# sunkafei/coffeedb

Hardware: AMD Instinct MI355X
Metric: sa_build_GiB_per_s (higher is better)
Workload: dtype u64

## Files before the change

coffeedb_amd/csrc/capi.hip:

```cpp
#include <dirent.h>

#include <algorithm>
#include <chrono>
#include <condition_variable>
#include <cstdlib>
#include <cstring>
#include <thread>

#include "../../include/coffeedb_gpu.h"
#include "index_impl.h"

using namespace cdb;

namespace {

double wall_ms() {
    using namespace std::chrono;
    return duration<double, std::milli>(steady_clock::now().time_since_epoch()).count();
}

void set_error(Index& ix, const char* msg) {
    std::lock_guard<std::mutex> g(ix.err_mu);
    ix.err = msg;
}
// ... 1467 lines not shown
        out->nrows = r.nrows;
        out->nhits = r.nhits;
        out->d_row_ptr = ix.q_rowptr.as<uint64_t>();
        out->d_ids = ix.q_ids.as<int64_t>();
        out->d_counts = ix.q_counts.as<int64_t>();
        if (hits) {
            hits->d_hit_ptr = ix.q_hitptr.as<uint64_t>();
            hits->d_offsets = ix.q_hitoff.as<uint64_t>();
        }
        ix.qstats.query_ms = wall_ms() - t0;
        ix.qstats.nhits = r.nhits;
        ix.qstats.nrows = r.nrows;
    });
}
}

int cdb_query_batch_device(cdb_index* h, const void* d_blob, const uint64_t* d_offsets, uint64_t npat,
                           uint64_t blob_bytes, cdb_device_result* out) {
    (void)blob_bytes;
    return query_batch_device_impl(h, d_blob, d_offsets, npat, out, nullptr);
}

int cdb_query_batch_offsets_device(cdb_index* h, const void* d_blob, const uint64_t* d_offsets, uint64_t npat,
                                   uint64_t blob_bytes, cdb_device_result* out, cdb_device_hits* hits) {
    (void)blob_bytes;
    if (!hits) return CDB_E_INVALID;
    return query_batch_device_impl(h, d_blob, d_offsets, npat, out, hits);
}

uint64_t cdb_size(const cdb_index* h) { return h ? h->ix.size : 0; }
uint64_t cdb_bits(const cdb_index* h) { return h ? h->ix.bits : 0; }
uint64_t cdb_mask(const cdb_index* h) { return h ? h->ix.mask : 0; }
int cdb_sa_width(const cdb_index* h) { return h ? h->ix.width : 0; }

int cdb_sa_copy(cdb_index* h, void* host_out, uint64_t capacity_bytes) {
    if (!h || !host_out) return CDB_E_INVALID;
    return guarded(h, [&] {
        Index& ix = h->ix;
        std::lock_guard<std::mutex> g(ix.mu);
        DeviceScope dscope(ix);
        const uint64_t need = ix.size * (uint64_t)ix.width;
        if (capacity_bytes < need) throw Error("cdb_sa_copy: buffer too small");
        if (need && ix.sa_packed) {
            DevBuf chunk;
            const uint64_t per = std::min<uint64_t>(ix.size, 32ull << 20);
            chunk.alloc(per * 8);
            for (uint64_t first = 0; first < ix.size; first += per) {
                const uint64_t cnt = std::min<uint64_t>(per, ix.size - first);
                sa_expand(ix, first, cnt, chunk.as<uint64_t>());
                CDB_HIP(hipMemcpyAsync(static_cast<char*>(host_out) + first * 8, chunk.p, cnt * 8, hipMemcpyDeviceToHost, ix.stream));
                CDB_HIP(hipStreamSynchronize(ix.stream));
            }
        } else if (need) {
            CDB_HIP(hipMemcpyAsync(host_out, ix.d_sa.p, need, hipMemcpyDeviceToHost, ix.stream));
            CDB_HIP(hipStreamSynchronize(ix.stream));
        }
    });
}

int cdb_set_option(cdb_index* h, const char* name, int64_t value) {
    if (!h || !name) return CDB_E_INVALID;
    Index& ix = h->ix;
    for (const char* o : {"fast_search", "key_directory", "single_query", "search_lanes", "keep_keys", "reference_compat"})
        if (!std::strcmp(name, o)) {
            std::lock_guard<std::mutex> g(ix.mu);
            query_resident_stop(ix);
        }
    if (!std::strcmp(name, "profile")) ix.prof.enabled = value != 0;
    else if (!std::strcmp(name, "reference_compat")) ix.reference_compat = value != 0;
    else if (!std::strcmp(name, "force_doubling")) ix.force_doubling = value != 0;
    else if (!std::strcmp(name, "initial_passes")) ix.initial_passes = (int)value;
    else if (!std::strcmp(name, "sort_variant")) ix.sort_variant = (int)value;
    else if (!std::strcmp(name, "keyhist3")) ix.keyhist3 = value != 0;
    else if (!std::strcmp(name, "key_symbols")) ix.key_symbols = (int)value;
    else if (!std::strcmp(name, "msd_first")) ix.msd_first = value != 0;
    else if (!std::strcmp(name, "msd_pair")) ix.msd_pair = value != 0;
    else if (!std::strcmp(name, "overlap_paircount")) ix.overlap_paircount = value != 0;
    else if (!std::strcmp(name, "key_directory")) { ix.key_directory = value != 0; ix.h_keydir.clear(); ix.keydir_tried = false; }
    else if (!std::strcmp(name, "fuse_records")) ix.fuse_records = value != 0;
    else if (!std::strcmp(name, "sweep_records")) ix.sweep_records = value != 0;
    else if (!std::strcmp(name, "partial_symbol")) ix.partial_symbol = value != 0;
    else if (!std::strcmp(name, "group_sort")) ix.group_sort = value != 0;
    else if (!std::strcmp(name, "list_rounds")) ix.list_rounds = value != 0;
    else if (!std::strcmp(name, "fuse_pairclass")) ix.fuse_pairclass = value != 0;
    else if (!std::strcmp(name, "group_sort_cap")) ix.group_sort_cap = (int)std::max<int64_t>(1, std::min<int64_t>(value, 1 << 20));
    else if (!std::strcmp(name, "vl_keys")) ix.vl_keys = value < 0 ? 0 : (value > 56 ? 56 : (int)value);
    else if (!std::strcmp(name, "pack_sa")) ix.pack_sa = value != 0;
    else if (!std::strcmp(name, "key_cost_model")) ix.key_cost_model = value != 0;
    else if (!std::strcmp(name, "gen_prebased")) ix.gen_prebased = value != 0;
    else if (!std::strcmp(name, "pack_entries")) ix.pack_entries = value != 0;
    else if (!std::strcmp(name, "segmented_sort")) ix.segmented_sort = value != 0;
    else if (!std::strcmp(name, "fold_root")) ix.fold_root = value != 0;
    else if (!std::strcmp(name, "fold_depth1")) ix.fold_depth1 = value != 0;
    else if (!std::strcmp(name, "flags_in_last_pass")) ix.flags_in_last_pass = value != 0;
    else if (!std::strcmp(name, "search_lanes")) ix.search_lanes = (value == 1 || value == 8) ? (int)value : 0;
    else if (!std::strcmp(name, "digit_bits")) ix.digit_bits = (int)value;
    else if (!std::strcmp(name, "fuse_keygen")) ix.fuse_keygen = value != 0;
    else if (!std::strcmp(name, "force_big_path")) ix.force_big_path = value != 0;
    else if (!std::strcmp(name, "debug_fail_build")) ix.debug_fail_build = value != 0;
    else if (!std::strcmp(name, "debug_no_segcap")) ix.debug_no_segcap = value != 0;
    else if (!std::strcmp(name, "debug_starve_group")) ix.debug_starve_group = (int)value;
    else if (!std::strcmp(name, "self_check")) ix.self_check = value < 0 ? 0 : value > 3 ? 3 : (int)value;
    else if (!std::strcmp(name, "premap_generation")) ix.premap_generation = value != 0;
    else if (!std::strcmp(name, "proof_cancel")) {
        if (value) proof_stop(ix);
    }
    else if (!std::strcmp(name, "debug_damage_after_build")) ix.debug_damage_after_build = value < 0 ? 0 : (uint64_t)value;
    else if (!std::strcmp(name, "debug_fail_self_check")) ix.debug_fail_self_check = value != 0;
    else if (!std::strcmp(name, "plain_tile_order")) ix.rws.plain_order = value != 0;
    else if (!std::strcmp(name, "key_coding")) ix.key_coding = (int)value;
    else if (!std::strcmp(name, "narrow_keys")) ix.narrow_keys = value != 0;
    else if (!std::strcmp(name, "single_query")) ix.use_single_query = value != 0;
    else if (!std::strcmp(name, "resident_query")) {
        std::lock_guard<std::mutex> g(ix.mu);
        if (value != 1) query_resident_stop(ix);
        ix.resident_mode = value <= 0 ? 0 : value == 1 ? 1 : 2;
        ix.resident_query = ix.resident_mode == 1;
        ix.single_streak = 0;
    }
    else if (!std::strcmp(name, "bucket_group_limit")) ix.bucket_group_limit = (uint64_t)value;
    else if (!std::strcmp(name, "query_hit_budget"))
        ix.query_hit_budget = value > 0 ? std::min<uint64_t>((uint64_t)value, 1ull << 31) : 1;
    else if (!std::strcmp(name, "coalesce_queries")) ix.coalesce_queries = value != 0;
    else if (!std::strcmp(name, "fast_search")) ix.use_fast_search = value != 0;
    else if (!std::strcmp(name, "wave_rows")) ix.use_wave_rows = value != 0;
    else if (!std::strcmp(name, "keep_keys")) ix.keep_keys = value != 0;
    else {
        set_error(ix, (std::string("unknown option: ") + name).c_str());
        return CDB_E_INVALID;
    }
    return CDB_OK;
}

int cdb_get_stat(const cdb_index* h, const char* name, double* value) {
    if (!h || !name || !value) return CDB_E_INVALID;
    const BuildStats& b = h->ix.bstats;
    const QueryStats& q = h->ix.qstats;
    struct { const char* n; double v; } tab[] = {
        {"build_ms", b.build_ms}, {"alloc_ms", b.alloc_ms}, {"free_ms", b.free_ms}, {"rounds", (double)b.rounds}, {"ext_rounds", (double)b.ext_rounds},
        {"dbl_rounds", (double)b.dbl_rounds}, {"unresolved_after_initial", (double)b.unresolved_initial},
        {"unresolved_max", (double)b.unresolved_max}, {"sort_passes", (double)b.sort_passes},
        {"sort_passes_skipped", (double)b.sort_passes_skipped}, {"isa_built", (double)b.isa_built}, {"fused_keygen", (double)b.fused_keygen}, {"dense_keys", (double)b.dense_keys}, {"key_layout", (double)b.key_layout}, {"bucketed", (double)b.bucketed}, {"bucket_groups", (double)b.bucket_groups}, {"segmented", (double)b.segmented}, {"fused_records", (double)b.fused_records}, {"sweep_records", (double)b.sweep_records}, {"vl_key_bits", (double)b.vl_key_bits}, {"partial_levels", (double)b.partial_levels}, {"list_rounds", (double)b.list_rounds}, {"pairclass_fused", (double)b.pairclass_fused}, {"group_sorts", (double)b.group_sorts}, {"group_sort_fallbacks", (double)b.group_sort_fallbacks}, {"vl_avg_len", b.vl_avg_len}, {"vl_rate", b.vl_rate}, {"vl_est_unresolved", b.vl_est_unresolved}, {"fixed_est_unresolved", b.fixed_est_unresolved}, {"gen_prebased", (double)b.gen_prebased}, {"root_folded", (double)b.root_folded}, {"flags_in_last_pass", (double)b.flags_in_last_pass}, {"msd_first", (double)b.msd_first}, {"bucket_low_digits", (double)b.bucket_low_digits}, {"key_directory_cells", h->ix.h_keydir.empty() ? 0.0 : (double)(h->ix.h_keydir.size() - 1)}, {"group_fallbacks", (double)h->ix.group_fallbacks}, {"dense_key_retries", (double)h->ix.dense_key_retries}, {"self_check_fallbacks", (double)h->ix.self_check_fallbacks}, {"sa_packed", h->ix.sa_packed ? 1.0 : 0.0}, {"sa_bytes_per_entry", h->ix.sa_packed ? 5.0 : (double)h->ix.width}, {"self_check_pairs", (double)h->ix.self_check_pairs}, {"self_check_ms", h->ix.self_check_ms}, {"self_check_coverage", h->ix.size > 1 ? (double)h->ix.self_check_pairs / (double)(h->ix.size - 1) : 0.0},
        {"order_proved", (h->ix.proof.state.load() == 2 || h->ix.proof.state.load() == 3 || (h->ix.self_check == 2 && h->ix.width != 0)) ? 1.0 : 0.0},
        {"proof_state", (double)h->ix.proof.state.load()}, {"proof_ms", h->ix.proof.ms}, {"proof_repair_ms", h->ix.proof.repair_ms},
        {"proof_pairs", (double)h->ix.proof.pairs}, {"proof_bad_pairs", (double)h->ix.proof.found[0]}, {"proof_invalid_entries", (double)h->ix.proof.found[1]}, {"proof_skipped_pairs", (double)h->ix.proof.skipped}, {"proof_mixed_pairs", (double)h->ix.proof.mixed},
        {"proof_runs", (double)h->ix.proof.runs}, {"pool_big_mallocs", (double)DevPool::get().big_mallocs()}, {"premap_ms", h->ix.proof.premap_ms}, {"premap_bytes", (double)h->ix.proof.premap_bytes},
        {"key_symbols", (double)b.key_symbols}, {"symbol_bits", (double)b.symbol_bits},
        {"alphabet", (double)b.alphabet}, {"digit_bits", (double)b.digit_bits}, {"final_depth", (double)b.final_depth}, {"compat_rotations", (double)b.compat_rotations},
        {"compat_depth", (double)b.compat_depth},
        {"host_upload_ms", h->ix.host_upload_ms}, {"host_free_ms", h->ix.host_free_ms},
        {"resident_answers", (double)h->ix.res_answers}, {"launched_answers", (double)h->ix.launched_answers}, {"resident_mode", (double)h->ix.resident_mode},
        {"cluster_table_bytes", h->ix.clu.valid ? (double)h->ix.clu.bytes() : 0.0}, {"cluster_classes", (double)h->ix.clu.nclasses},
        {"cluster_prepare_ms", h->ix.clu.prepare_ms}, {"cluster_ms", h->ix.clu.last_ms}, {"cluster_resorted", h->ix.clu.resorted ? 1.0 : 0.0},
        {"query_ms", q.query_ms}, {"query_upload_ms", q.upload_ms}, {"query_device_ms", q.device_ms}, {"query_download_ms", q.download_ms}, {"query_hits", (double)q.nhits}, {"query_rows", (double)q.nrows},
    };
    for (auto& e : tab)
        if (!std::strcmp(e.n, name)) {
            *value = e.v;
            return CDB_OK;
        }
    return CDB_E_INVALID;
}

int cdb_profile_get(cdb_index* h, const char* kernel, double* total_ms, uint64_t* launches, uint64_t* bytes) {
    if (!h || !kernel) return CDB_E_INVALID;
    std::lock_guard<std::mutex> g(h->ix.mu);
    auto it = h->ix.prof.recs.find(kernel);
    if (it == h->ix.prof.recs.end()) return CDB_E_INVALID;
    if (total_ms) *total_ms = it->second.ms;
    if (launches) *launches = it->second.launches;
    if (bytes) *bytes = it->second.bytes;
    return CDB_OK;
}

int cdb_profile_dump(cdb_index* h, char* buf, size_t cap) {
    if (!h || !buf || cap == 0) return CDB_E_INVALID;
    std::lock_guard<std::mutex> g(h->ix.mu);
    std::string s;
    for (auto& kv : h->ix.prof.recs) {
        char line[256];
        std::snprintf(line, sizeof(line), "%s %.6f %llu %llu\n", kv.first.c_str(), kv.second.ms,
                      (unsigned long long)kv.second.launches, (unsigned long long)kv.second.bytes);
        s += line;
    }
    std::strncpy(buf, s.c_str(), cap - 1);
    buf[cap - 1] = 0;
    return CDB_OK;
}

int cdb_debug_verify(cdb_index* h, uint64_t out[5]) {
    if (!h || !out) return CDB_E_INVALID;
    return guarded(h, [&] {
        Index& ix = h->ix;
        std::lock_guard<std::mutex> g(ix.mu);
        DeviceScope dscope(ix);
        if (ix.width == 0) throw Error("index has not been built");
        verify_suffix_array(ix, out);
    });
}

int cdb_debug_self_check(cdb_index* h, int full, uint64_t out[2]) {
    if (!h || !out) return CDB_E_INVALID;
    return guarded(h, [&] {
        Index& ix = h->ix;
        std::lock_guard<std::mutex> g(ix.mu);
        DeviceScope dscope(ix);
        if (ix.width == 0) throw Error("index has not been built");
        spot_check_suffix_array(ix, full ? 0u : (uint32_t)std::min<uint64_t>(1u << 15, ix.size > 1 ? ix.size - 1 : 1), out);
    });
}

int cdb_proof_wait(cdb_index* h, double timeout_ms) {
    if (!h) return CDB_E_INVALID;
    const double t0 = wall_ms();
    for (;;) {
        const int st = h->ix.proof.state.load();
        if (st != 1 && !h->ix.proof.busy.load(std::memory_order_acquire)) return st;
        if (timeout_ms >= 0 && wall_ms() - t0 >= timeout_ms) return st;
        std::this_thread::sleep_for(std::chrono::microseconds(200));
    }
}

int cdb_debug_verify_reference(cdb_index* h, uint64_t out[4]) {
    if (!h || !out) return CDB_E_INVALID;
// ... 125 lines not shown
```

coffeedb_amd/csrc/common.h:

```cpp
#pragma once
#include <hip/hip_runtime.h>

#include <algorithm>
#include <atomic>
#include <cstdint>
#include <cstdio>
#include <cstdlib>
#include <cstring>
#include <map>
#include <mutex>
#include <stdexcept>
#include <string>
#include <vector>

namespace cdb {

struct Error : std::runtime_error {
    using std::runtime_error::runtime_error;
};
struct RetryWithDenseKeys : Error {
    using Error::Error;
};

#define CDB_HIP(expr)                                                                            \
// ... 346 lines not shown
        std::lock_guard<std::mutex> g(mu_);
        live_[p] = need;
        return p;
    }
    bool release(void* p) {
        size_t bytes;
        {
            std::lock_guard<std::mutex> g(mu_);
            auto it = live_.find(p);
            if (it == live_.end()) return false;
            bytes = it->second;
            live_.erase(it);
            if (cached_ + bytes <= limit_) {
                free_.push_back(Block{p, bytes});
                cached_ += bytes;
                return true;
            }
        }
        (void)hipHostFree(p);
        return true;
    }
    void trim() {
        std::vector<Block> blocks;
        {
            std::lock_guard<std::mutex> g(mu_);
            blocks.swap(free_);
            cached_ = 0;
        }
        for (auto& b : blocks) (void)hipHostFree(b.p);
    }
    size_t cached_bytes() {
        std::lock_guard<std::mutex> g(mu_);
        return cached_;
    }

private:
    struct Block { void* p; size_t bytes; };
    std::mutex mu_;
    std::vector<Block> free_;
    std::map<void*, size_t> live_;
    size_t cached_ = 0;
    size_t limit_ = 8ull << 30;
};

inline void* host_alloc(size_t bytes, bool zero = false) {
    if (bytes == 0) bytes = 8;
    void* p = bytes >= HostPool::kMinPinned ? HostPool::get().alloc(bytes) : nullptr;
    if (!p) p = std::malloc(bytes);
    if (!p) throw std::bad_alloc();
    if (zero) std::memset(p, 0, bytes);
    return p;
}
inline void host_free(void* p) {
    if (p && !HostPool::get().release(p)) std::free(p);
}

struct Profiler {
    struct Rec { double ms = 0; uint64_t launches = 0; uint64_t bytes = 0; };
    struct Pending { std::string name; hipEvent_t a, b; uint64_t bytes; };
    bool enabled = false;
    std::map<std::string, Rec> recs;
    std::vector<Pending> pending;
    std::vector<hipEvent_t> pool;

    hipEvent_t get_event() {
        if (!pool.empty()) { hipEvent_t e = pool.back(); pool.pop_back(); return e; }
        hipEvent_t e;
        CDB_HIP(hipEventCreate(&e));
        return e;
    }
    int begin(hipStream_t s) {
        if (!enabled) return -1;
        Pending p{"", get_event(), get_event(), 0};
        CDB_HIP(hipEventRecord(p.a, s));
        pending.push_back(p);
        return (int)pending.size() - 1;
    }
    void end(int tok, const char* name, uint64_t bytes, hipStream_t s) {
        if (tok < 0) return;
        pending[tok].name = name;
        pending[tok].bytes = bytes;
        CDB_HIP(hipEventRecord(pending[tok].b, s));
    }
    void resolve() {
        for (auto& p : pending) {
            float ms = 0;
            if (hipEventElapsedTime(&ms, p.a, p.b) == hipSuccess) {
                Rec& r = recs[p.name];
                r.ms += ms;
                r.launches += 1;
                r.bytes += p.bytes;
            }
            pool.push_back(p.a);
            pool.push_back(p.b);
        }
        pending.clear();
    }
    void reset() { recs.clear(); }
    ~Profiler() {
        for (auto& p : pending) { (void)hipEventDestroy(p.a); (void)hipEventDestroy(p.b); }
        for (auto e : pool) (void)hipEventDestroy(e);
    }
};

}
```

coffeedb_amd/csrc/index_impl.h:

```cpp
#pragma once
#include <atomic>
#include <condition_variable>
#include <mutex>
#include <thread>
#include <string>
#include <vector>

#include "../../include/coffeedb_gpu.h"
#include "common.h"
#include "radix_sort.h"

namespace cdb {

constexpr int TEXT_PAD = 128;

struct BuildStats {
    double build_ms = 0, alloc_ms = 0, free_ms = 0;
    int rounds = 0;
    int ext_rounds = 0;
    int dbl_rounds = 0;
    uint64_t unresolved_initial = 0;
    uint64_t unresolved_max = 0;
    int sort_passes = 0;
    int sort_passes_skipped = 0;
    int isa_built = 0;
    int fused_keygen = 0;
    int key_layout = 0;
    int dense_keys = 0;
    int bucketed = 0;
    int bucket_low_digits = 0;
    int bucket_groups = 0;
    int root_folded = 0;
    int flags_in_last_pass = 0;
    int msd_first = 0;
    int gen_prebased = 0;
    int fused_records = 0;
    int sweep_records = 0;
    int pairclass_fused = 0;
    int list_rounds = 0;
    int group_sorts = 0, group_sort_fallbacks = 0;
    int partial_levels = 0;
    int vl_key_bits = 0;
    double vl_avg_len = 0, vl_rate = 0, vl_est_unresolved = 0, fixed_est_unresolved = 0;
    int segmented = 0;
    uint64_t gather_items = 0;
    int key_symbols = 0, symbol_bits = 0, alphabet = 0, digit_bits = 8;
    uint64_t final_depth = 0;
    uint64_t compat_rotations = 0, compat_depth = 0;
};

struct QueryStats {
    double query_ms = 0;
    double upload_ms = 0, device_ms = 0, download_ms = 0;
    uint64_t nhits = 0, nrows = 0;
};

struct SingleKeys {
    const uint64_t* keys64 = nullptr;
    const uint32_t* keys32 = nullptr;
    const void* keylow = nullptr;
    int low_bits = 0, low_bytes = 0, nsym = 0;
    bool decisive = false;
    uint64_t klo = 0, khi = 0;
    bool ranged = false;
    uint64_t lo0 = 0, hi0 = 0;
};

struct Sa40 {
    const uint32_t* __restrict__ lo;
    const uint8_t* __restrict__ hi;
    __device__ __forceinline__ uint64_t operator[](uint64_t i) const { return (uint64_t)lo[i] | ((uint64_t)hi[i] << 32); }
};
struct Packed40 {};
template <typename T> struct SaOf {
    using val = T;
    using ptr = const T* __restrict__;
};
template <> struct SaOf<Packed40> {
    using val = uint64_t;
    using ptr = Sa40;
};
template <typename V> struct SaRW {
    V* p;
    using val = V;
    __device__ __forceinline__ V load(uint64_t i) const { return p[i]; }
    __device__ __forceinline__ void store(uint64_t i, V v) const { p[i] = v; }
};
struct Sa40RW {
    uint32_t* lo;
    uint8_t* hi;
    using val = uint64_t;
    __device__ __forceinline__ uint64_t load(uint64_t i) const { return (uint64_t)lo[i] | ((uint64_t)hi[i] << 32); }
    __device__ __forceinline__ void store(uint64_t i, uint64_t v) const {
        lo[i] = (uint32_t)v;
        hi[i] = (uint8_t)(v >> 32);
    }
};

struct Index {
    int device = 0;
    hipStream_t stream = nullptr;
    std::mutex mu;
    std::mutex qmu;
    std::condition_variable qcv;
    std::vector<void*> qpending;
    bool qleader = false;
    bool coalesce_queries = true;
    bool keep_keys = true;
    bool use_wave_rows = true;
    bool use_single_query = true;
    void* h_single = nullptr;
    void* d_single = nullptr;
    int resident_mode = 2;
    bool resident_query = false;
    uint32_t single_streak = 0;
    int64_t last_single_ns = 0;
    uint64_t res_answers = 0, launched_answers = 0;
    void* h_res = nullptr;
    void* d_res = nullptr;
    hipStream_t res_stream = nullptr;
    hipStream_t aux_stream = nullptr;
    hipEvent_t aux_ev[2] = {nullptr, nullptr};
// ... 1 lines not shown
    bool res_running = false;
    uint32_t res_seq = 0;
    SingleKeys res_keys;
    bool use_fast_search = true;

    std::vector<int64_t> ids;
    std::vector<uint64_t> doc_start{0};
    std::string host_text;
    bool host_tables_valid = true;
    bool host_text_valid = true;

    uint64_t bits = 1, mask = 1, size = 0;
    int off_bits = 1;
    int width = 0;
    uint64_t ndocs = 0;

    DevBuf d_text_owned;
    const uint8_t* d_text = nullptr;
    bool text_padded = false;
    DevBuf d_doc_start;
    DevBuf d_ids;
    DevBuf d_sa;
    DevBuf d_sa_hi;
    bool sa_packed = false;
    bool gen_prebased = true;
    TileBaseWorkspace tbw;
    bool key_cost_model = true;
    bool pack_sa = true;
    void release_sa() {
        d_sa.release();
        d_sa_hi.release();
        sa_packed = false;
        clu.drop();
    }
    template <typename T> typename SaOf<T>::ptr sa_view() const;
    bool sa_sorted = false;
    DevBuf d_keys;
    DevBuf d_symmap_q;
    uint16_t h_symmap_q[256] = {};
    DevBuf d_keys32, d_keylow;
    int key_low_bits = 0;
    int key_low_bytes = 0;
    int key_nsym = 0;
    uint32_t key_base = 0;
    void drop_keys() {
        d_keys.release();
        d_keys32.release();
        d_keylow.release();
        key_nsym = 0;
        key_low_bits = 0;
        key_low_bytes = 0;
        h_keydir.clear();
        h_keydir.shrink_to_fit();
        keydir_tried = false;
    }
    std::vector<uint32_t> h_keydir;
    int keydir_shift = 0, keydir_bits = 0;
    bool keydir_tried = false;
    bool key_directory = true;
    DevBuf d_pivots;
    int pivot_levels = 0;

    RadixWorkspace rws;
    MsdWorkspace msd_ws;
    DevBuf scan_partials;
    uint64_t q_spec_cap = 0;
    DevBuf q_spec;
    DevBuf q_pat, q_offs, q_left, q_right, q_hoff, q_keys0, q_keys1, q_flags, q_rowptr, q_ids, q_counts, q_hitptr, q_hitoff;

    bool reference_compat = true;
    bool force_doubling = false;
    int initial_passes = 0;
    int key_symbols = 0;
    int sort_variant = 0;
    int search_lanes = 0;
    bool flags_in_last_pass = true;
    bool fold_depth1 = true;
    bool fold_root = true;
    bool segmented_sort = true;
    bool fuse_records = true;
    bool fuse_pairclass = true;
    bool list_rounds = true;
    int group_sort_cap = 4096;
    bool group_sort = true;
    bool partial_symbol = true;
    int vl_keys = 2;
    bool vl_off_once = false;
    bool sweep_records = true;
    bool pack_entries = true;
    bool msd_first = true;
    bool msd_pair = true;
    bool keyhist3 = true;
    int dense_key_retries = 0;
    int group_fallbacks = 0;
    uint64_t bucket_group_limit = 0;
    uint64_t self_check_pairs = 0;
    double self_check_ms = 0;
    int self_check = 3;
    int self_check_fallbacks = 0;
    bool debug_fail_self_check = false;
    struct Proof {
        std::thread th;
        std::atomic<int> state{0};
        std::atomic<bool> cancel{false};
        hipStream_t stream = nullptr;
        void* d_out = nullptr;
        double ms = 0, repair_ms = 0;
        uint64_t pairs = 0;
        uint64_t found[2] = {0, 0};
        uint64_t skipped = 0;
        uint64_t mixed = 0;
        uint64_t runs = 0;
        bool of_loaded_file = false;
        std::atomic<bool> busy{false};
        bool want_proof = false;
        double premap_ms = 0;
        uint64_t premap_bytes = 0;
    } proof;
    bool premap_generation = false;
    bool proof_in_repair = false;
    uint64_t debug_damage_after_build = 0;
    bool debug_no_segcap = false;
    int debug_starve_group = 0;
    bool debug_fail_build = false;
    bool force_big_path = false;
    bool fuse_keygen = true;
    int digit_bits = 0;
    bool narrow_keys = true;
    int key_coding = 0;
    uint64_t query_hit_budget = 1ull << 31;

    struct ClusterTables {
        bool valid = false;
        uint64_t nclasses = 0;
        bool ids_ascend = true;
        bool resorted = false;
        DevBuf class_of_doc;
        DevBuf class_rep;
        DevBuf id_sorted, id_doc;
        double prepare_ms = 0, last_ms = 0;
        uint64_t bytes() const { return class_of_doc.bytes + class_rep.bytes + id_sorted.bytes + id_doc.bytes; }
        void drop() {
            valid = false;
            nclasses = 0;
            class_of_doc.release();
            class_rep.release();
            id_sorted.release();
            id_doc.release();
        }
    } clu;

    double host_upload_ms = 0, host_free_ms = 0;
    Profiler prof;
    BuildStats bstats;
    QueryStats qstats;
    mutable std::mutex err_mu;
    std::string err;
};

void ensure_host_tables(Index& ix);
void ensure_host_staging(Index& ix);

void read_raw_dir(const char* dir, const char* key, std::vector<int64_t>& ids, std::vector<uint64_t>& doc_start, std::string& text,
                  uint64_t& nrec, uint64_t& nadd);

void build_suffix_array(Index& ix);
// ... 122 lines not shown
```

coffeedb_amd/csrc/sa_build.hip:

```cpp
#include <algorithm>
#include <chrono>
#include <cmath>
#include <cstdlib>
#include <cstring>

#include "index_impl.h"
#include "records_sweep.h"
#include "vl_code.h"
#include "scan.h"

#ifndef RS_GATHER_ABL
#define RS_GATHER_ABL 0
#endif

namespace cdb {
namespace {

constexpr int KG_TILE = 2048;
constexpr int KG_LOOK = 64;

__global__ __launch_bounds__(256) void sa_bytecount_kernel(const uint8_t* __restrict__ text, uint64_t n,
                                                           unsigned long long* __restrict__ counts) {
    __shared__ uint32_t s[256];
    s[threadIdx.x] = 0;
// ... 1220 lines not shown
    const uint64_t g = kbits >= 64 ? 0ull : k >> kbits;
    auto gid = [&](uint64_t x) { return kbits >= 64 ? 0ull : x >> kbits; };
    uint64_t pos = j;
    uint32_t walked = 0;
    bool too = false;
    {
        uint32_t d = 1;
        for (; d <= cap && j >= d; ++d) {
            const uint64_t o = kin[j - d];
            if (gid(o) != g) break;
            pos -= (uint64_t)(o > k);
            if ((d & 127u) == 0 && vstate[0]) return;
        }
        too = d > cap && j >= d && gid(kin[j - d]) == g;
        walked += d - 1;
    }
    if (!too) {
        uint32_t d = 1;
        for (; d <= cap && j + d < m; ++d) {
            const uint64_t o = kin[j + d];
            if (gid(o) != g) break;
            pos += (uint64_t)(o < k);
            if ((d & 127u) == 0 && vstate[0]) return;
        }
        too = d > cap && j + d < m && gid(kin[j + d]) == g;
        walked += d - 1;
    }
    if (walked > GS_FREE && !too) too = atomicAdd(&state[1], (unsigned long long)walked) + walked > budget;
    if (too) {
        atomicExch(&state[0], 1ull);
        return;
    }
    kout[pos] = k;
    vout[pos] = vin[j];
}

template <typename I>
__global__ __launch_bounds__(256) void sa_newhead_kernel(const uint64_t* __restrict__ skey, const I* __restrict__ U,
                                                         const uint8_t* __restrict__ flags, uint64_t m,
                                                         uint8_t* __restrict__ nh) {
    const uint64_t j = (uint64_t)blockIdx.x * 256 + threadIdx.x;
    if (j >= m) return;
    const bool oldhead = flags[U[j]] & 1;
    nh[j] = (uint8_t)(oldhead || j == 0 || skey[j] != skey[j - 1]);
}

template <typename SAW, typename I, bool WANT_POS = true>
__device__ __forceinline__ void sa_place(uint64_t j, uint64_t m, const typename SAW::val* sval, const I* U, const uint8_t* nh,
                                         const uint64_t* doc_start, int bits, uint64_t mask, uint64_t hnew, SAW sa,
                                         uint8_t* flags, uint64_t& ext_pos, unsigned long long* still_open,
                                         const uint8_t* hcov = nullptr, uint32_t h_add = 0, uint8_t* lf = nullptr) {
    if (hcov) hnew = (uint64_t)hcov[j] + h_add;
    const typename SAW::val v = sval[j];
    const uint64_t i = U[j];
    const bool head = nh[j];
    const bool last = j + 1 == m || nh[j + 1];
    const uint64_t d = (uint64_t)v & mask, off = (uint64_t)v >> bits;
    uint64_t ds = 0;
    bool exhausted = false;
    if (WANT_POS || !(head && last)) {
        ds = doc_start[d];
        exhausted = doc_start[d + 1] - ds - off < hnew;
    }
    const bool open = !(head && last) && !exhausted;
    sa.store(i, v);
    flags[i] = (uint8_t)((head ? 1 : 0) | (open ? 2 : 0));
    if (lf) lf[j] = (uint8_t)((head ? 1 : 0) | (open ? 2 : 0));
    if (open) atomicAdd(still_open, 1ull);
    ext_pos = ds + d + off;
}

template <typename SAW, typename I>
__global__ __launch_bounds__(256) void sa_update_kernel(const typename SAW::val* __restrict__ sval, const I* __restrict__ U,
                                                        const uint8_t* __restrict__ nh, uint64_t m,
                                                        const uint64_t* __restrict__ doc_start, int bits,
                                                        uint64_t mask, uint64_t hnew, SAW sa,
                                                        uint8_t* __restrict__ flags,
                                                        unsigned long long* __restrict__ still_open,
                                                        const uint8_t* __restrict__ hcov = nullptr, uint32_t h_add = 0, uint8_t* __restrict__ lf = nullptr) {
    const uint64_t j = (uint64_t)blockIdx.x * 256 + threadIdx.x;
    if (j >= m) return;
    uint64_t q;
    sa_place<SAW, I, false>(j, m, sval, U, nh, doc_start, bits, mask, hnew, sa, flags, q, still_open, hcov, h_add, lf);
}

template <typename I>
struct HeadIn {
    const uint8_t* nh;
    const I* U;
    __device__ __forceinline__ uint64_t operator()(uint64_t j) const { return nh[j] ? (uint64_t)U[j] + 1 : 0ull; }
};
struct SlotOrder {
    const unsigned long long* a_start = nullptr;
    const unsigned long long* u_start = nullptr;
    uint32_t nseg = 0;
    __device__ __forceinline__ uint64_t operator()(uint64_t slot) const {
        if (nseg == 0) return slot;
        uint32_t lo = 0, hi = nseg - 1;
        while (lo < hi) {
            const uint32_t mid = lo + (hi - lo + 1) / 2;
            if (a_start[mid] <= slot) lo = mid; else hi = mid - 1;
        }
        return slot - a_start[lo] + u_start[lo];
    }
};

template <typename SAW, typename I, typename R>
struct UpdateOut {
    using V = typename SAW::val;
    const V* sval;
    const I* U;
    const uint8_t* nh;
    uint64_t m;
    const uint64_t* doc_start;
    int bits;
    uint64_t mask, hnew;
    SAW sa;
    uint8_t* flags;
    R* rank;
    unsigned long long* still_open;
    SlotOrder order;
    __device__ __forceinline__ void operator()(uint64_t j, uint64_t, uint64_t incl) const {
        uint64_t q;
        sa_place<SAW, I>(j, m, sval, U, nh, doc_start, bits, mask, hnew, sa, flags, q, still_open);
        rank[q] = (R)(order(incl - 1) + 1);
    }
};

struct AllHeadIn {
    const uint8_t* flags;
    __device__ __forceinline__ uint64_t operator()(uint64_t i) const { return (flags[i] & 1) ? i + 1 : 0ull; }
};
template <typename SAW, typename R>
struct IsaOut {
    SAW sa;
    const uint64_t* doc_start;
    int bits;
    uint64_t mask;
    R* rank;
    SlotOrder order;
    __device__ __forceinline__ void operator()(uint64_t i, uint64_t, uint64_t incl) const {
        const auto v = sa.load(i);
        const uint64_t d = (uint64_t)v & mask, off = (uint64_t)v >> bits;
        rank[doc_start[d] + d + off] = (R)(order(incl - 1) + 1);
    }
};

struct CompatBucket {
    unsigned long long lo, hi;
};

template <typename V>
__global__ __launch_bounds__(320) void compat_bounds_kernel(typename SaOf<V>::ptr sa,
                                                            const uint8_t* __restrict__ text,
                                                            const uint64_t* __restrict__ doc_start, int bits,
                                                            uint64_t mask, const CompatBucket* __restrict__ buckets,
                                                            uint64_t depth, unsigned long long* __restrict__ bounds) {
    const int c = threadIdx.x;
    if (c > 257) return;
    const CompatBucket b = buckets[blockIdx.x];
    uint64_t lo = b.lo, hi = b.hi;
    if (c == 257) {
        bounds[(uint64_t)blockIdx.x * 258 + c] = b.hi;
        return;
    }
    while (lo < hi) {
// ... 1629 lines not shown
        ix.key_nsym = kp.nsym;
        ix.key_base = kp.kbase;
    } else {
        is.sorted_keys.release();
        is.sorted_k32.release();
        is.sorted_low.release();
    }
    ix.bstats.free_ms += now_ms() - ta;
}

struct RefineBuffers {
    DevBuf d_order;
    DevBuf U, skey[2], sval[2], nh, rank, hcov;
    DevBuf d_open;
    DevBuf U2b, lf;
    DevBuf d_gs_state;
};

SlotOrder make_slot_order(Index& ix, const InitialSort& is, const Alphabet& al, DevBuf& d_order) {
    SlotOrder order;
    if (is.folded_roots.empty()) return order;
    const std::vector<Depth1Fold>& depth1 = is.depth1;
    struct Blk { unsigned long long a, len; int code, cls; };
    std::vector<Blk> blks;
    std::vector<int> code_of_root;
    {
        for (int b = 128; b < 256; ++b) if (al.h_map[b]) code_of_root.push_back(al.h_map[b]);
        for (int b = 0; b < 128; ++b) if (al.h_map[b]) code_of_root.push_back(al.h_map[b]);
    }
    for (size_t b = 0; b < is.folded_roots.size(); ++b) {
        const CompatBucket r = is.folded_roots[b];
        if (!depth1.empty() && depth1[b].done) {
            blks.push_back(Blk{r.lo, depth1[b].nend, code_of_root[b], 0});
            blks.push_back(Blk{r.lo + depth1[b].nend, depth1[b].nhigh, code_of_root[b], 2});
            blks.push_back(Blk{r.lo + depth1[b].nend + depth1[b].nhigh, depth1[b].nlow, code_of_root[b], 1});
        } else {
            blks.push_back(Blk{r.lo, r.hi - r.lo, code_of_root[b], 0});
        }
    }
    std::vector<size_t> by_u(blks.size());
    for (size_t i = 0; i < by_u.size(); ++i) by_u[i] = i;
    std::sort(by_u.begin(), by_u.end(), [&](size_t x, size_t y) {
        return blks[x].code != blks[y].code ? blks[x].code < blks[y].code : blks[x].cls < blks[y].cls;
    });
    std::vector<unsigned long long> tab(2 * blks.size());
    unsigned long long at = 0;
    for (size_t i : by_u) {
        tab[blks.size() + i] = at;
        at += blks[i].len;
    }
    for (size_t i = 0; i < blks.size(); ++i) tab[i] = blks[i].a;
    d_order.alloc(tab.size() * sizeof(unsigned long long));
    CDB_HIP(hipMemcpyAsync(d_order.p, tab.data(), tab.size() * sizeof(unsigned long long), hipMemcpyHostToDevice, ix.stream));
    CDB_HIP(hipStreamSynchronize(ix.stream));
    order.a_start = d_order.as<unsigned long long>();
    order.u_start = d_order.as<unsigned long long>() + blks.size();
    order.nseg = (uint32_t)blks.size();
    return order;
}

template <typename V, typename I, typename R, typename SAW>
uint64_t refine_groups(Index& ix, SAW sa, InitialSort& is, const Alphabet& al, const KeyPlan& kp, SortStats& ss, RefineBuffers& rb) {
    hipStream_t s = ix.stream;
    const uint64_t n = ix.size, D = ix.ndocs;
    BuildStats& st = ix.bstats;
    const uint8_t* text = ix.d_text;
    const uint64_t* doc_start = ix.d_doc_start.as<uint64_t>();
    const int symbits = al.symbits;
    const DevBuf& flags = is.flags;
    const uint32_t vl_kb1 = is.vl_kb1;
    const SlotOrder order = make_slot_order(ix, is, al, rb.d_order);
    DevBuf &U = rb.U, (&skey)[2] = rb.skey, (&sval)[2] = rb.sval, &nh = rb.nh, &rank = rb.rank, &hcov = rb.hcov;
    DevBuf &d_open = rb.d_open, &U2b = rb.U2b, &lf = rb.lf, &d_gs_state = rb.d_gs_state;
    uint32_t h_acc = 0;
    uint64_t h = is.refine_depth0 ? is.refine_depth0 : (uint64_t)kp.nsym;
    bool isa = false;
    uint64_t cap = 0;
    d_open.alloc(sizeof(uint64_t));
    bool have_list = false;
    uint64_t m_list = 0;
    int list_rs = 0;
    d_gs_state.alloc(2 * sizeof(unsigned long long));
    bool group_sort_on = ix.group_sort;
    for (;;) {
        if (st.rounds > 0) {
            uint64_t still = 0;
            CDB_HIP(hipMemcpyAsync(&still, d_open.p, sizeof(still), hipMemcpyDeviceToHost, s));
            CDB_HIP(hipStreamSynchronize(s));
            if (still == 0) break;
        }
        CDB_HIP(hipMemsetAsync(d_open.p, 0, sizeof(uint64_t), s));
        auto flag_tile_sums = [&]() {
            const uint64_t nb = ceil_div(n, SC_TILE);
            ix.scan_partials.ensure(scan_partials_slots(nb) * sizeof(U2));
            int t = ix.prof.begin(s);
            hipLaunchKernelGGL(sa_flag_count_kernel, dim3((unsigned)ceil_div(nb, (uint64_t)(4 * FC_TILES_PER_WAVE))), dim3(256), 0, s,
                               (const uint8_t*)flags.as<uint8_t>(), n, nb, ix.scan_partials.as<U2>());
            ix.prof.end(t, "sa_flag_count", n, s);
        };
        bool from_list = have_list && ix.list_rounds;
        have_list = false;
        if (from_list) {
            const uint64_t nb = ceil_div(m_list, SC_TILE);
            ix.scan_partials.ensure(scan_partials_slots(nb) * sizeof(U2));
            int t = ix.prof.begin(s);
            hipLaunchKernelGGL(sa_flag_count_kernel, dim3((unsigned)ceil_div(nb, (uint64_t)(4 * FC_TILES_PER_WAVE))), dim3(256), 0, s,
                               (const uint8_t*)lf.as<uint8_t>(), m_list, nb, ix.scan_partials.as<U2>());
            ix.prof.end(t, "sa_flag_count", m_list, s);
        } else if (!is.tile_sums_ready) {
            flag_tile_sums();
        }
        U2 tot = scan_totals_from_partials<U2>(s, ix.scan_partials, from_list ? m_list : n, OpAdd{}, U2{0, 0});
        is.tile_sums_ready = false;
        uint64_t m = tot.a, G = tot.b;
        if (st.rounds == 0) st.unresolved_initial = m;
        st.unresolved_max = std::max(st.unresolved_max, m);
        if (m == 0) break;
        if (m >= (1ull << 32) - 4096) throw Error("too many unresolved suffixes for one refinement round (internal limit: 2^32)");
        const int gbits = bit_width64(G - 1);
        int nsym2 = std::min((64 - gbits) / symbits, KG_LOOK);
        if (!isa) {
            const bool use_text = !ix.force_doubling && nsym2 >= 1 &&
                                  ((m <= n / 32 && st.ext_rounds < 4) || (m <= n / 8 && st.ext_rounds < 2));
            if (!use_text) {
                rank.alloc((n + D + 1) * sizeof(R));
                CDB_HIP(hipMemsetAsync(rank.p, 0, (n + D + 1) * sizeof(R), s));
                AllHeadIn ain{flags.as<uint8_t>()};
                (void)scan_totals<uint64_t>(s, ix.scan_partials, ain, n, OpMax{}, (uint64_t)0);
                IsaOut<SAW, R> iout{sa, doc_start, (int)ix.bits, ix.mask, rank.as<R>(), order};
                int t = ix.prof.begin(s);
                scan_apply<uint64_t>(s, ix.scan_partials, ain, n, OpMax{}, (uint64_t)0, iout);
                ix.prof.end(t, "sa_isa_init", n * (1 + sizeof(V) + sizeof(R)), s);
                isa = true;
                st.isa_built = 1;
                from_list = false;
                flag_tile_sums();
                (void)scan_totals_from_partials<U2>(s, ix.scan_partials, n, OpAdd{}, U2{0, 0});
            }
        }
        const int kbits = isa ? bit_width64(n) : nsym2 * symbits;
        if (kbits + gbits > 64) throw Error("refinement key does not fit 64 bits (internal limit)");
        if (m > cap) {
            cap = m;
            U.alloc(m * sizeof(I));
            skey[0].alloc(m * 8);
            skey[1].alloc(m * 8);
            sval[0].alloc(m * sizeof(V));
            sval[1].alloc(m * sizeof(V));
            nh.alloc(m);
            lf.alloc(m + 16);
            if (vl_kb1) hcov.alloc(m);
        }
        {
            int t = ix.prof.begin(s);
            if (from_list) {
                if (list_rs == 0) {
                    std::swap(skey[0], skey[1]);
                    std::swap(sval[0], sval[1]);
                    list_rs = 1;
                }
                U2b.ensure(cap * sizeof(I));
                CompactListOut<V, I> co{(const I*)U.as<I>(), (const V*)sval[1].as<V>(), U2b.as<I>(), skey[0].as<uint64_t>(), sval[0].as<V>(), kbits};
                hipLaunchKernelGGL((sa_flag_compact_kernel<decltype(co)>), dim3((unsigned)ceil_div(ceil_div(m_list, SC_TILE), (uint64_t)(4 * FC_TILES_PER_WAVE))),
                                   dim3(256), 0, s, (const uint8_t*)lf.as<uint8_t>(), m_list, (uint64_t)ceil_div(m_list, SC_TILE),
                                   (const U2*)ix.scan_partials.as<U2>(), co);
                std::swap(U, U2b);
                st.list_rounds++;
            } else {
            CompactOut<SAW, I> co{sa, U.as<I>(), skey[0].as<uint64_t>(), sval[0].as<V>(), kbits};
            hipLaunchKernelGGL((sa_flag_compact_kernel<decltype(co)>), dim3((unsigned)ceil_div(ceil_div(n, SC_TILE), (uint64_t)(4 * FC_TILES_PER_WAVE))),
                               dim3(256), 0, s, (const uint8_t*)flags.as<uint8_t>(), n, (uint64_t)ceil_div(n, SC_TILE),
                               (const U2*)ix.scan_partials.as<U2>(), co);
            }
            if (isa)
                hipLaunchKernelGGL((sa_round_keys_kernel<V, R, true>), dim3((unsigned)ceil_div(m, 256)), dim3(256), 0, s,
                                   (const V*)sval[0].as<V>(), m, doc_start, text, (const uint16_t*)al.d_symmap.as<uint16_t>(),
                                   (const R*)rank.as<R>(), (int)ix.bits, ix.mask, h, nsym2, symbits, skey[0].as<uint64_t>(), n);
            else
                hipLaunchKernelGGL((sa_round_keys_kernel<V, R, false>), dim3((unsigned)ceil_div(m, 256)), dim3(256), 0, s,
                                   (const V*)sval[0].as<V>(), m, doc_start, text, (const uint16_t*)al.d_symmap.as<uint16_t>(),
                                   (const R*)nullptr, (int)ix.bits, ix.mask, h, nsym2, symbits, skey[0].as<uint64_t>(), n,
                                   vl_kb1 ? (const uint8_t*)is.d_vl_bytelen.as<uint8_t>() : nullptr, vl_kb1, h_acc, vl_kb1 ? hcov.as<uint8_t>() : nullptr);
            ix.prof.end(t, "sa_compact", n + m * (sizeof(I) + 8 + 2 * sizeof(V)), s);
        }
        int rs = -1;
        if (group_sort_on) {
            CDB_HIP(hipMemsetAsync(d_gs_state.p, 0, 2 * sizeof(unsigned long long), s));
            int t = ix.prof.begin(s);
            hipLaunchKernelGGL((sa_group_sort_kernel<V>), dim3((unsigned)ceil_div(m, 256)), dim3(256), 0, s, (const uint64_t*)skey[0].as<uint64_t>(),
                               (const V*)sval[0].as<V>(), m, kbits, (uint32_t)ix.group_sort_cap, (unsigned long long)(16 * m + (1u << 20)),
                               skey[1].as<uint64_t>(), sval[1].as<V>(), d_gs_state.as<unsigned long long>());
            ix.prof.end(t, "sa_group_sort", m * 2 * (8 + sizeof(V)), s);
            unsigned long long gave_up = 0;
            CDB_HIP(hipMemcpyAsync(&gave_up, d_gs_state.p, sizeof(gave_up), hipMemcpyDeviceToHost, s));
            CDB_HIP(hipStreamSynchronize(s));
            if (gave_up) {
                group_sort_on = false;
                st.group_sort_fallbacks++;
// ... 252 lines not shown
```

Before: 29.94.

## Settle small unresolved suffix groups in-register before refinement rounds

Adds a wave-level settle pass that, before the refinement loop, takes small unresolved groups (up to a cap of 64) and resolves them in registers by extending text keys and ranking within the group via lane shuffles and permutes. A second kernel handles groups that straddle 4096-flag tile edges. The aim is to shrink the unresolved set cheaply so later global sort and refinement rounds handle fewer suffixes or are skipped. It adds an extra flag-count scan up front, two kernel launches and per-group divergent work, and if few groups are small this is pure overhead.

Result: slower. 26.57 (-11.3%).

```diff
diff --git a/coffeedb_amd/csrc/capi.hip b/coffeedb_amd/csrc/capi.hip
--- a/coffeedb_amd/csrc/capi.hip
+++ b/coffeedb_amd/csrc/capi.hip
@@ -1573,6 +1573,9 @@
     else if (!std::strcmp(name, "partial_symbol")) ix.partial_symbol = value != 0;
     else if (!std::strcmp(name, "group_sort")) ix.group_sort = value != 0;
     else if (!std::strcmp(name, "list_rounds")) ix.list_rounds = value != 0;
+    else if (!std::strcmp(name, "settle_small")) ix.settle_small = value != 0;
+    else if (!std::strcmp(name, "settle_cap")) ix.settle_cap = (int)std::max<int64_t>(1, std::min<int64_t>(value, 64));
+    else if (!std::strcmp(name, "settle_iters")) ix.settle_iters = (int)std::max<int64_t>(1, std::min<int64_t>(value, 16));
     else if (!std::strcmp(name, "fuse_pairclass")) ix.fuse_pairclass = value != 0;
     else if (!std::strcmp(name, "group_sort_cap")) ix.group_sort_cap = (int)std::max<int64_t>(1, std::min<int64_t>(value, 1 << 20));
     else if (!std::strcmp(name, "vl_keys")) ix.vl_keys = value < 0 ? 0 : (value > 56 ? 56 : (int)value);
@@ -1630,7 +1633,8 @@
     struct { const char* n; double v; } tab[] = {
         {"build_ms", b.build_ms}, {"alloc_ms", b.alloc_ms}, {"free_ms", b.free_ms}, {"rounds", (double)b.rounds}, {"ext_rounds", (double)b.ext_rounds},
         {"dbl_rounds", (double)b.dbl_rounds}, {"unresolved_after_initial", (double)b.unresolved_initial},
-        {"unresolved_max", (double)b.unresolved_max}, {"sort_passes", (double)b.sort_passes},
+        {"unresolved_max", (double)b.unresolved_max}, {"settled_in_place", (double)b.settled_in_place}, {"settle_left", (double)b.settle_left},
+{"sort_passes", (double)b.sort_passes},
         {"sort_passes_skipped", (double)b.sort_passes_skipped}, {"isa_built", (double)b.isa_built}, {"fused_keygen", (double)b.fused_keygen}, {"dense_keys", (double)b.dense_keys}, {"key_layout", (double)b.key_layout}, {"bucketed", (double)b.bucketed}, {"bucket_groups", (double)b.bucket_groups}, {"segmented", (double)b.segmented}, {"fused_records", (double)b.fused_records}, {"sweep_records", (double)b.sweep_records}, {"vl_key_bits", (double)b.vl_key_bits}, {"partial_levels", (double)b.partial_levels}, {"list_rounds", (double)b.list_rounds}, {"pairclass_fused", (double)b.pairclass_fused}, {"group_sorts", (double)b.group_sorts}, {"group_sort_fallbacks", (double)b.group_sort_fallbacks}, {"vl_avg_len", b.vl_avg_len}, {"vl_rate", b.vl_rate}, {"vl_est_unresolved", b.vl_est_unresolved}, {"fixed_est_unresolved", b.fixed_est_unresolved}, {"gen_prebased", (double)b.gen_prebased}, {"root_folded", (double)b.root_folded}, {"flags_in_last_pass", (double)b.flags_in_last_pass}, {"msd_first", (double)b.msd_first}, {"bucket_low_digits", (double)b.bucket_low_digits}, {"key_directory_cells", h->ix.h_keydir.empty() ? 0.0 : (double)(h->ix.h_keydir.size() - 1)}, {"group_fallbacks", (double)h->ix.group_fallbacks}, {"dense_key_retries", (double)h->ix.dense_key_retries}, {"self_check_fallbacks", (double)h->ix.self_check_fallbacks}, {"sa_packed", h->ix.sa_packed ? 1.0 : 0.0}, {"sa_bytes_per_entry", h->ix.sa_packed ? 5.0 : (double)h->ix.width}, {"self_check_pairs", (double)h->ix.self_check_pairs}, {"self_check_ms", h->ix.self_check_ms}, {"self_check_coverage", h->ix.size > 1 ? (double)h->ix.self_check_pairs / (double)(h->ix.size - 1) : 0.0},
         {"order_proved", (h->ix.proof.state.load() == 2 || h->ix.proof.state.load() == 3 || (h->ix.self_check == 2 && h->ix.width != 0)) ? 1.0 : 0.0},
         {"proof_state", (double)h->ix.proof.state.load()}, {"proof_ms", h->ix.proof.ms}, {"proof_repair_ms", h->ix.proof.repair_ms},
diff --git a/coffeedb_amd/csrc/common.h b/coffeedb_amd/csrc/common.h
--- a/coffeedb_amd/csrc/common.h
+++ b/coffeedb_amd/csrc/common.h
@@ -452,6 +452,9 @@
         pending[tok].bytes = bytes;
         CDB_HIP(hipEventRecord(pending[tok].b, s));
     }
+    void add_bytes(int tok, uint64_t bytes) {
+        if (tok >= 0 && (size_t)tok < pending.size()) pending[tok].bytes += bytes;
+    }
     void resolve() {
         for (auto& p : pending) {
             float ms = 0;
diff --git a/coffeedb_amd/csrc/index_impl.h b/coffeedb_amd/csrc/index_impl.h
--- a/coffeedb_amd/csrc/index_impl.h
+++ b/coffeedb_amd/csrc/index_impl.h
@@ -38,6 +38,7 @@
     int sweep_records = 0;
     int pairclass_fused = 0;
     int list_rounds = 0;
+    uint64_t settled_in_place = 0, settle_left = 0;
     int group_sorts = 0, group_sort_fallbacks = 0;
     int partial_levels = 0;
     int vl_key_bits = 0;
@@ -205,6 +206,9 @@
     bool fuse_pairclass = true;
     bool list_rounds = true;
     int group_sort_cap = 4096;
+    bool settle_small = true;
+    int settle_cap = 64;
+    int settle_iters = 3;
     bool group_sort = true;
     bool partial_symbol = true;
     int vl_keys = 2;
diff --git a/coffeedb_amd/csrc/sa_build.hip b/coffeedb_amd/csrc/sa_build.hip
--- a/coffeedb_amd/csrc/sa_build.hip
+++ b/coffeedb_amd/csrc/sa_build.hip
@@ -1326,6 +1326,230 @@
     if (j >= m) return;
     uint64_t q;
     sa_place<SAW, I, false>(j, m, sval, U, nh, doc_start, bits, mask, hnew, sa, flags, q, still_open, hcov, h_add, lf);
+}
+
+template <typename SAW>
+struct SettleCtx {
+    SAW sa;
+    uint8_t* flags;
+    const uint8_t* text;
+    uint64_t n_text;
+    const uint64_t* doc_start;
+    const uint16_t* symmap;
+    int bits;
+    uint64_t mask;
+    uint32_t h0;
+    int nsym, symbits;
+    uint32_t cap, iters;
+    const uint8_t* vl_len;
+    uint32_t vl_kb1;
+    unsigned long long* settled;
+};
+
+__device__ __forceinline__ uint32_t ss_push(uint32_t to_lane, uint32_t x) {
+    return (uint32_t)__builtin_amdgcn_ds_permute((int)(to_lane << 2), (int)x);
+}
+__device__ __forceinline__ uint64_t ss_push64(uint32_t to_lane, uint64_t x) {
+    return (uint64_t)ss_push(to_lane, (uint32_t)x) | ((uint64_t)ss_push(to_lane, (uint32_t)(x >> 32)) << 32);
+}
+__device__ __forceinline__ uint64_t ss_shfl64(uint64_t x, uint32_t from_lane) {
+    return (uint64_t)(uint32_t)__shfl((int)(uint32_t)x, (int)from_lane) | ((uint64_t)(uint32_t)__shfl((int)(uint32_t)(x >> 32), (int)from_lane) << 32);
+}
+__device__ __forceinline__ void ss_bounds(uint64_t hb, int lane, uint32_t cut, uint32_t& gs, uint32_t& ge) {
+    const uint64_t upto = lane == 63 ? ~0ull : (2ull << lane) - 1ull;
+    gs = 63u - (uint32_t)__clzll((long long)(hb & upto));
+    const uint64_t above = hb & ~upto;
+    ge = above ? (uint32_t)__ffsll((long long)above) - 1u : cut;
+}
+
+template <typename SAW>
+__device__ __forceinline__ void settle_trip(const SettleCtx<SAW>& c, int lane, uint64_t i, uint64_t hb, uint32_t cut) {
+    using V = typename SAW::val;
+    const bool live = (uint32_t)lane < cut;
+    uint32_t gs, ge;
+    ss_bounds(hb, lane, cut, gs, ge);
+    const bool act = live && ge - gs <= c.cap;
+    if (__builtin_amdgcn_ballot_w64(act) == 0) return;
+    bool open = act, head = live && ((hb >> lane) & 1ull);
+    V v = 0;
+    uint64_t p0 = 0;
+    uint32_t len = 0, hl = c.h0;
+    if (act) {
+        v = c.sa.load(i);
+        const uint64_t d = (uint64_t)v & c.mask, off = (uint64_t)v >> c.bits;
+        const uint64_t ds = c.doc_start[d];
+        const uint64_t L = c.doc_start[d + 1] - ds - off;
+        p0 = ds + off;
+        len = (uint32_t)(L < 0x7FFFFFFFull ? L : 0x7FFFFFFFull);
+        if (c.vl_len) {
+            const uint8_t* q = c.text + p0;
+            const uint64_t pa = (uint64_t)q & ~7ull;
+            const uint32_t sh = (uint32_t)((uint64_t)q & 7ull) * 8u;
+            const uint64_t tend = (uint64_t)(c.text + c.n_text);
+            const uint64_t w0 = *reinterpret_cast<const uint64_t*>(pa);
+            const uint64_t w1 = pa + 8 < tend ? *reinterpret_cast<const uint64_t*>(pa + 8) : 0ull;
+            const uint64_t w2 = pa + 16 < tend ? *reinterpret_cast<const uint64_t*>(pa + 16) : 0ull;
+            const uint64_t b0 = sh ? (w0 >> sh) | (w1 << (64u - sh)) : w0;
+            const uint64_t b1 = sh ? (w1 >> sh) | (w2 << (64u - sh)) : w1;
+            uint32_t used = 0, cov = 1;
+            while ((uint64_t)cov < L && cov < 200u) {
+                const uint32_t byte = cov < 8u ? (uint32_t)(b0 >> (8u * cov)) & 0xFFu : (cov < 16u ? (uint32_t)(b1 >> (8u * (cov - 8u))) & 0xFFu : (uint32_t)q[cov]);
+                used += c.vl_len[byte];
+                if (used > c.vl_kb1) break;
+                ++cov;
+            }
+            hl = cov;
+        }
+    }
+    for (uint32_t it = 0; it < c.iters; ++it) {
+        if (__builtin_amdgcn_ballot_w64(open) == 0) break;
+        uint64_t key = 0;
+        if (open && len > hl) {
+            const uint32_t rem = len - hl;
+            const uint8_t* p = c.text + p0 + hl;
+            const uint64_t pa = (uint64_t)p & ~7ull;
+            const uint32_t sh = (uint32_t)((uint64_t)p & 7ull) * 8u;
+            const uint64_t w0 = *reinterpret_cast<const uint64_t*>(pa);
+            const uint64_t w1 = pa + 8 < (uint64_t)(c.text + c.n_text) ? *reinterpret_cast<const uint64_t*>(pa + 8) : 0ull;
+            const uint64_t lo = sh ? (w0 >> sh) | (w1 << (64u - sh)) : w0;
+            const uint32_t b8 = (uint32_t)(w1 >> sh) & 0xFFu;
+            for (int k = 0; k < c.nsym; ++k) {
+                const uint32_t byte = k < 8 ? (uint32_t)(lo >> (8 * k)) & 0xFFu : b8;
+                const uint64_t sym = (uint32_t)k < rem ? (uint64_t)c.symmap[byte] : 0ull;
+                key = (key << c.symbits) | sym;
+            }
+        }
+        ss_bounds(hb, lane, cut, gs, ge);
+        const uint32_t size = ge - gs;
+        uint32_t less = 0, eqf = 0;
+        for (uint32_t dd = 0; __builtin_amdgcn_ballot_w64(open && dd < size) != 0; ++dd) {
+            const uint32_t src = gs + dd < 64u ? gs + dd : 63u;
+            const uint64_t ok = ss_shfl64(key, src);
+            if (open && dd < size) {
+                less += (uint32_t)(ok < key);
+                eqf += (uint32_t)(ok == key && src < (uint32_t)lane);
+            }
+        }
+        const uint32_t to = open ? gs + less + eqf : (uint32_t)lane;
+        const uint32_t nhd = open ? (uint32_t)(eqf == 0) : (uint32_t)head;
+        if constexpr (sizeof(V) == 4) v = (V)ss_push(to, (uint32_t)v);
+        else v = (V)ss_push64(to, (uint64_t)v);
+        p0 = ss_push64(to, p0);
+        len = ss_push(to, len);
+        head = ss_push(to, nhd) != 0;
+        hb = __builtin_amdgcn_ballot_w64(live && head);
+        hl += (uint32_t)c.nsym;
+        ss_bounds(hb, lane, cut, gs, ge);
+        if (open) open = ge - gs > 1 && len >= hl;
+    }
+    if (act) {
+        c.sa.store(i, v);
+        c.flags[i] = (uint8_t)((head ? 1 : 0) | (open ? 2 : 0));
+    }
+    const uint64_t done = __builtin_amdgcn_ballot_w64(act && !open);
+    if (lane == 0 && done) atomicAdd(c.settled, (unsigned long long)__popcll(done));
+}
+
+template <typename SAW>
+__global__ __launch_bounds__(256) void sa_settle_small_kernel(SettleCtx<SAW> c, uint64_t n, uint64_t tiles) {
+    static_assert(SC_TILE == 4096, "flag sweep assumes 4096-flag tiles");
+    __shared__ uint16_t s_list[4][SC_TILE];
+    const int lane = threadIdx.x & 63, wave = threadIdx.x >> 6;
+    uint16_t* const list = s_list[wave];
+    const uint64_t t0 = ((uint64_t)blockIdx.x * 4 + wave) * FC_TILES_PER_WAVE;
+    for (uint32_t k = 0; k < FC_TILES_PER_WAVE; ++k) {
+        const uint64_t tile = t0 + k;
+        if (tile >= tiles) break;
+        const uint64_t tbase = tile * SC_TILE;
+        uint32_t x[4][4], v[4], incl[4];
+#pragma unroll
+        for (int q = 0; q < 4; ++q) fc_load(c.flags, n, tbase + (uint64_t)q * 1024 + (uint64_t)lane * 16, x[q]);
+#pragma unroll
+        for (int q = 0; q < 4; ++q) incl[q] = v[q] = fc_count(x[q]);
+#pragma unroll
+        for (int off = 1; off < 64; off <<= 1) {
+#pragma unroll
+            for (int q = 0; q < 4; ++q) {
+                const uint32_t y = __shfl_up(incl[q], off);
+                if (lane >= off) incl[q] += y;
+            }
+        }
+        uint32_t any = 0;
+#pragma unroll
+        for (int q = 0; q < 4; ++q) any |= v[q];
+        if (__builtin_amdgcn_ballot_w64(any != 0) == 0) continue;
+        uint32_t cpre = 0;
+#pragma unroll
+        for (int q = 0; q < 4; ++q) {
+            const uint32_t ctot = __shfl(incl[q], 63);
+            if (v[q] & 0xFFFFu) {
+                uint32_t slot = (cpre + incl[q] - v[q]) & 0xFFFFu;
+                uint32_t um = 0, hm = 0;
+#pragma unroll
+                for (int w = 0; w < 4; ++w) {
+                    const uint32_t u = (x[q][w] >> 1) & 0x01010101u;
+                    um |= (((u * 0x01020408u) >> 24) & 0xFu) << (4 * w);
+                    hm |= ((((u & x[q][w]) * 0x01020408u) >> 24) & 0xFu) << (4 * w);
+                }
+                const uint32_t off0 = (uint32_t)q * 1024u + (uint32_t)lane * 16u;
+                while (um) {
+                    const uint32_t b = (uint32_t)__builtin_ctz(um);
+                    um &= um - 1u;
+                    list[slot++] = (uint16_t)((off0 + b) | (((hm >> b) & 1u) << 12));
+                }
+            }
+            cpre += ctot;
+        }
+        const uint32_t total = cpre & 0xFFFFu;
+        __builtin_amdgcn_fence(__ATOMIC_RELEASE, "wavefront");
+        __builtin_amdgcn_wave_barrier();
+        __builtin_amdgcn_fence(__ATOMIC_ACQUIRE, "wavefront");
+        const bool straddle = total > 0 && ((uint32_t)list[total - 1] & 0xFFFu) == SC_TILE - 1 && tbase + SC_TILE < n &&
+                              !(c.flags[tbase + SC_TILE] & 1);
+        uint32_t b0 = 0;
+        while (b0 < total) {
+            const uint32_t t = b0 + (uint32_t)lane;
+            const uint32_t e = t < total ? (uint32_t)list[t] : 0u;
+            const uint64_t hbm = __builtin_amdgcn_ballot_w64(((e >> 12) & 1u) != 0);
+            if (!(hbm & 1ull)) {
+                b0 += hbm ? (uint32_t)__builtin_ctzll(hbm) : 64u;
+                continue;
+            }
+            const uint32_t nl = total - b0 < 64u ? total - b0 : 64u;
+            const bool complete = b0 + 64u < total ? (((uint32_t)list[b0 + 64u] >> 12) & 1u) != 0 : !straddle;
+            const uint32_t cut = complete ? nl : 63u - (uint32_t)__builtin_clzll(hbm);
+            if (cut == 0) {
+                b0 += nl;
+                continue;
+            }
+            settle_trip(c, lane, tbase + (uint64_t)(e & 0xFFFu), cut >= 64u ? hbm : hbm & ((1ull << cut) - 1ull), cut);
+            b0 += cut;
+        }
+        __builtin_amdgcn_fence(__ATOMIC_RELEASE, "wavefront");
+        __builtin_amdgcn_wave_barrier();
+    }
+}
+
+template <typename SAW>
+__global__ __launch_bounds__(256) void sa_settle_edges_kernel(SettleCtx<SAW> c, uint64_t n, uint64_t tiles) {
+    const int lane = threadIdx.x & 63, wave = threadIdx.x >> 6;
+    const uint64_t first = (((uint64_t)blockIdx.x * 4 + wave) * 64ull + 1ull);
+    const uint64_t mine = (first + (uint64_t)lane) * SC_TILE;
+    const bool st = first + (uint64_t)lane < tiles && mine < n && c.flags[mine] == 2;
+    uint64_t todo = __builtin_amdgcn_ballot_w64(st);
+    while (todo) {
+        const uint32_t which = (uint32_t)__builtin_ctzll(todo);
+        todo &= todo - 1ull;
+        const uint64_t b = (first + which) * SC_TILE;
+        const uint32_t fa = c.flags[b - 64 + (uint64_t)lane];
+        const uint32_t fb = b + (uint64_t)lane < n ? (uint32_t)c.flags[b + (uint64_t)lane] : 1u;
+        const uint64_t ha = __builtin_amdgcn_ballot_w64((fa & 1u) != 0), hbn = __builtin_amdgcn_ballot_w64((fb & 1u) != 0);
+        if (!ha || !hbn) continue;
+        const uint32_t hl = 63u - (uint32_t)__builtin_clzll(ha);
+        const uint32_t len = 64u - hl + (uint32_t)__builtin_ctzll(hbn);
+        if (len > 64u) continue;
+        settle_trip(c, lane, b - 64 + hl + (uint64_t)lane, 1ull, len);
+    }
 }
 
 template <typename I>
@@ -3121,6 +3345,41 @@
     int list_rs = 0;
     d_gs_state.alloc(2 * sizeof(unsigned long long));
     bool group_sort_on = ix.group_sort;
+    auto flag_tile_sums = [&]() {
+        const uint64_t nb = ceil_div(n, SC_TILE);
+        ix.scan_partials.ensure(scan_partials_slots(nb) * sizeof(U2));
+        int t = ix.prof.begin(s);
+        hipLaunchKernelGGL(sa_flag_count_kernel, dim3((unsigned)ceil_div(nb, (uint64_t)(4 * FC_TILES_PER_WAVE))), dim3(256), 0, s,
+                           (const uint8_t*)flags.as<uint8_t>(), n, nb, ix.scan_partials.as<U2>());
+        ix.prof.end(t, "sa_flag_count", n, s);
+    };
+    bool have_tot = false;
+    U2 tot0{0, 0};
+    bool settled = false;
+    unsigned long long h_settled = 0;
+    int settle_tok = -1;
+    if (ix.settle_small && !ix.force_doubling) {
+        if (!is.tile_sums_ready) flag_tile_sums();
+        tot0 = scan_totals_from_partials<U2>(s, ix.scan_partials, n, OpAdd{}, U2{0, 0});
+        is.tile_sums_ready = false;
+        have_tot = true;
+        st.unresolved_initial = tot0.a;
+        st.unresolved_max = std::max(st.unresolved_max, (uint64_t)tot0.a);
+        if (tot0.a > 0 && tot0.a <= n / 8) {
+            SettleCtx<SAW> sc{sa, flags.as<uint8_t>(), text, n, doc_start, (const uint16_t*)al.d_symmap.as<uint16_t>(), (int)ix.bits, ix.mask,
+                              (uint32_t)h, std::max(1, std::min(64 / symbits, 9)), symbits, (uint32_t)ix.settle_cap, (uint32_t)ix.settle_iters,
+                              vl_kb1 ? (const uint8_t*)is.d_vl_bytelen.as<uint8_t>() : nullptr, vl_kb1, d_open.as<unsigned long long>()};
+            const uint64_t nb = ceil_div(n, SC_TILE);
+            CDB_HIP(hipMemsetAsync(d_open.p, 0, sizeof(uint64_t), s));
+            settle_tok = ix.prof.begin(s);
+            hipLaunchKernelGGL((sa_settle_small_kernel<SAW>), dim3((unsigned)ceil_div(nb, (uint64_t)(4 * FC_TILES_PER_WAVE))), dim3(256), 0, s, sc, n, nb);
+            if (nb > 1) hipLaunchKernelGGL((sa_settle_edges_kernel<SAW>), dim3((unsigned)ceil_div(nb - 1, (uint64_t)256)), dim3(256), 0, s, sc, n, nb);
+            ix.prof.end(settle_tok, "sa_settle_small", n, s);
+            CDB_HIP(hipMemcpyAsync(&h_settled, d_open.p, sizeof(h_settled), hipMemcpyDeviceToHost, s));
+            settled = true;
+            have_tot = false;
+        }
+    }
     for (;;) {
         if (st.rounds > 0) {
             uint64_t still = 0;
@@ -3129,17 +3388,10 @@
             if (still == 0) break;
         }
         CDB_HIP(hipMemsetAsync(d_open.p, 0, sizeof(uint64_t), s));
-        auto flag_tile_sums = [&]() {
-            const uint64_t nb = ceil_div(n, SC_TILE);
-            ix.scan_partials.ensure(scan_partials_slots(nb) * sizeof(U2));
-            int t = ix.prof.begin(s);
-            hipLaunchKernelGGL(sa_flag_count_kernel, dim3((unsigned)ceil_div(nb, (uint64_t)(4 * FC_TILES_PER_WAVE))), dim3(256), 0, s,
-                               (const uint8_t*)flags.as<uint8_t>(), n, nb, ix.scan_partials.as<U2>());
-            ix.prof.end(t, "sa_flag_count", n, s);
-        };
         bool from_list = have_list && ix.list_rounds;
         have_list = false;
-        if (from_list) {
+        if (have_tot) {
+        } else if (from_list) {
             const uint64_t nb = ceil_div(m_list, SC_TILE);
             ix.scan_partials.ensure(scan_partials_slots(nb) * sizeof(U2));
             int t = ix.prof.begin(s);
@@ -3149,10 +3401,18 @@
         } else if (!is.tile_sums_ready) {
             flag_tile_sums();
         }
-        U2 tot = scan_totals_from_partials<U2>(s, ix.scan_partials, from_list ? m_list : n, OpAdd{}, U2{0, 0});
+        U2 tot = have_tot ? tot0 : scan_totals_from_partials<U2>(s, ix.scan_partials, from_list ? m_list : n, OpAdd{}, U2{0, 0});
+        have_tot = false;
         is.tile_sums_ready = false;
         uint64_t m = tot.a, G = tot.b;
-        if (st.rounds == 0) st.unresolved_initial = m;
+        if (st.rounds == 0 && settled) {
+            st.settled_in_place = h_settled;
+            st.settle_left = m;
+            ix.prof.add_bytes(settle_tok, h_settled * (2 * (std::is_same<SAW, Sa40RW>::value ? 5 : sizeof(V)) + 1 + 64));
+        } else if (st.rounds == 0) {
+            st.unresolved_initial = m;
+            if (ix.settle_small) st.settle_left = m;
+        }
         st.unresolved_max = std::max(st.unresolved_max, m);
         if (m == 0) break;
         if (m >= (1ull << 32) - 4096) throw Error("too many unresolved suffixes for one refinement round (internal limit: 2^32)");
```
